# Chanuk-Yang/Deep_Continuous_Fusion_for_Multi-Sensor_3D_Object_Detection

Hardware: AMD Instinct MI355X
Metric: frames/sec (train step) 100k-pt LiDAR + 1242x375 RGB (higher is better)
Workload: dtype bf16; 1 GPU; cfg2: grid 32x704x800, 100000 pts/frame, 1242x375 RGB, ResNet-18 image stream, K=3 fusion x4 sites, eval-mode BN (reference F4), batch 2/GPU; global_batch=2, parallelism=dp1, loss_sampling=compat, conv_chain=False

## Files before the change

### deep_continuous_fusion_for_multi-sensor_3d_object_detection_amd/_hip.py

```python
import ctypes
import os
import subprocess

import numpy as np
import torch

_HERE = os.path.dirname(os.path.abspath(__file__))
LIB_PATH = os.environ.get("DCF_HIP_LIB") or os.path.join(_HERE, "libdcf_hip.so")
CSRC = os.path.join(_HERE, "csrc")

F32, BF16, F16 = 0, 1, 2
VOXEL_COMPAT, VOXEL_ACCUM, VOXEL_COMPAT_ROUNDS, VOXEL_OCCUPANCY = 0, 1, 2, 3
PROJ_COMPAT, PROJ_CORRECT = 0, 1

c_int, c_float, c_i64, c_size_t, c_void_p = ctypes.c_int, ctypes.c_float, ctypes.c_int64, ctypes.c_size_t, ctypes.c_void_p
P = c_void_p

SIGNATURES = {
    "dcf_last_error": (ctypes.c_char_p, []),
    "dcf_version": (c_int, []),
    "dcf_set_option": (c_int, [ctypes.c_char_p, ctypes.c_char_p]),
    "dcf_prof_enable": (c_int, [c_int]),
    "dcf_prof_reset": (c_int, []),
    "dcf_prof_calibrate": (c_int, [P, c_int]),
    "dcf_prof_read": (c_int, [P, P, P, P, c_int]),
    "dcf_prof_read2": (c_int, [P, P, P, P, P, c_int]),
    "dcf_compact_workspace_bytes": (c_size_t, [c_int]),
    "dcf_range_filter": (c_int, [P, c_int, P, P, P, P, P, P]),
    "dcf_voxelize_workspace_bytes": (c_size_t, [c_int, c_int, c_int]),
    "dcf_voxelize": (c_int, [P, c_int, P, P, c_int, c_int, c_int, c_int, P, P, P]),
    "dcf_voxelize_batch": (c_int, [P, P, c_int, P, P, c_int, c_int, c_int, P, P, P]),
    "dcf_voxelize_batch_nhwc": (c_int, [c_int, P, P, c_int, P, P, c_int, c_int, c_int, P, P, P]),
    "dcf_project_filter": (c_int, [P, c_int, P, P, c_float, c_float, c_int, P, P, P, P, P, P]),
    "dcf_project_filter_batch": (c_int, [P, P, c_int, P, P, c_float, c_float, c_int, P, P, c_int, P, P, P]),
    "dcf_knn_workspace_bytes": (c_size_t, [c_int, c_int, c_int]),
    "dcf_knn_bev": (c_int, [P, P, c_int, c_int, c_int, c_int, c_int, c_float, c_float, c_float, c_float, c_float, P, P, P]),
    "dcf_knn_bev_batch": (c_int, [P, P, c_int, c_int, c_int, c_int, c_int, c_int, c_float, c_float, c_float, c_float, c_float, P, P, c_size_t, P]),
    "dcf_knn_bev_sites": (c_int, [P, P, c_int, c_int, c_int, P, c_int, c_float, c_float, c_float, c_float, c_float, P]),
    "dcf_knn_bev_batch_shared": (c_int, [P, P, c_int, c_int, c_int, c_int, c_int, c_int, c_int, c_int, c_int, c_float, c_float, c_float, c_float, c_float, P, P, c_size_t, P, c_size_t, P]),
    "dcf_nchw_to_nhwc": (c_int, [c_int, P, P, c_int, c_int, c_int, c_int, P]),
    "dcf_nhwc_to_nchw": (c_int, [c_int, P, P, c_int, c_int, c_int, c_int, P]),
    "dcf_image_to_nhwc4": (c_int, [c_int, P, P, c_int, c_int, c_int, P]),
    "dcf_conv2d_fwd": (c_int, [c_int, P, P, P, P, P] + [c_int] * 12 + [P]),
    "dcf_conv2d_fwd_rowscale": (c_int, [c_int, P, P, P, P, P, P] + [c_int] * 12 + [P]),
    "dcf_conv2d_dgrad": (c_int, [c_int, P, P, P, P, P] + [c_int] * 11 + [P]),
    "dcf_conv2d_dgrad_halfres": (c_int, [c_int, P, P, P, P, P, P] + [c_int] * 11 + [P]),
    "dcf_conv3x3_chain_supported": (c_int, [c_int] * 6),
    "dcf_conv3x3_chain_workspace_bytes": (c_size_t, [c_int] * 6),
    "dcf_conv3x3_chain": (c_int, [c_int, P, c_int, c_int, c_int, c_int, c_int, c_int, P, P]),
    "dcf_fp8_act_scale": (c_int, [c_float, P]),
    "dcf_cast_fp8": (c_int, [c_int, P, P, P, P, c_i64, P]),
    "dcf_weight_prep_fp8": (c_int, [P, P, c_int, c_int, P, P, P, P, P, c_float, P]),
    "dcf_conv2d_fwd_fp8": (c_int, [c_int, P, P, P, P, P, P, P, P, P, P] + [c_int] * 12 + [P]),
    "dcf_conv2d_wgrad_splits": (c_int, [c_int] * 8),
    "dcf_conv2d_wgrad": (c_int, [c_int, P, P, P, P, c_int] + [c_int] * 11 + [P]),
    "dcf_conv2d_wgrad_groupable": (c_int, [c_int] * 10),
    "dcf_conv2d_wgrad_group": (c_int, [P, c_int, P]),
    "dcf_stem7x7_fwd": (c_int, [c_int, P, P, P, P] + [c_int] * 7 + [P]),
    "dcf_stem7x7_wgrad": (c_int, [c_int, P, P, P, P, c_int] + [c_int] * 6 + [P]),
    "dcf_weight_prep": (c_int, [c_int, P, c_int, P, P, P, P, c_float, P]),
    "dcf_wgrad_finalize": (c_int, [P, c_int, c_int, P, P, P, P, P, P, c_float, P]),
    "dcf_eval_score_filter": (c_int, [P, c_int, c_int, c_int, c_float, c_int, P, P, P]),
    "dcf_eval_nms_workspace_bytes": (c_size_t, [c_int]),
    "dcf_eval_nms": (c_int, [P, P, c_int, c_int, ctypes.c_double, P, P, P, P]),
    "dcf_eval_match": (c_int, [P, c_int, P, c_int, P, c_int, P, P]),
    "dcf_wgrad_finalize_rows": (c_int, [P, c_int, P, P, P, P, P, P, P, c_float, P]),
    "dcf_bn_workspace_bytes": (c_size_t, [c_int]),
    "dcf_bn_train_fwd": (c_int, [c_int, P, P, P, P, P, P, P, P, P, c_i64, c_int, c_float, c_float, c_int, P, P]),
    "dcf_bn_train_bwd": (c_int, [c_int, P, P, P, P, P, P, P, P, c_i64, c_int, P, P]),
    "dcf_relu_bwd_chansum": (c_int, [c_int, P, P, P, c_i64, c_int, c_int, P]),
    "dcf_resize_bilinear_fwd": (c_int, [c_int, P, P, P] + [c_int] * 7 + [P]),
    "dcf_resize_bilinear_bwd": (c_int, [c_int, P, P] + [c_int] * 7 + [P]),
    "dcf_maxpool3x3s2_fwd": (c_int, [c_int, P, P] + [c_int] * 6 + [P]),
    "dcf_maxpool3x3s2_bwd": (c_int, [c_int, P, P, P, P] + [c_int] * 6 + [P]),
    "dcf_maxpool3x3s2_fwd_idx": (c_int, [c_int, P, P, P] + [c_int] * 6 + [P]),
    "dcf_maxpool3x3s2_bwd_idx": (c_int, [c_int, P, P, P] + [c_int] * 6 + [P]),
    "dcf_head_fwd": (c_int, [c_int, P, c_int, P, P, c_int, c_int, c_int, P]),
    "dcf_head_bwd": (c_int, [c_int, P, c_int, P, P, P, P, c_int, c_int, c_int, P]),
    "dcf_point_sample_fwd": (c_int, [c_int, P, c_int, c_int, c_int, P, P, c_int, P, P]),
    "dcf_point_sample_bwd": (c_int, [c_int, P, c_int, c_int, c_int, P, P, c_int, P, P]),
    "dcf_point_sample_fwd_batch": (c_int, [c_int, P, c_int, c_int, c_int, P, c_i64, P, c_int, P, c_int, P]),
    "dcf_point_sample_bwd_batch": (c_int, [c_int, P, c_int, c_int, c_int, P, c_i64, P, c_int, P, c_int, P]),
    "dcf_fusion_gather_fwd_batch": (c_int, [c_int, P, c_i64, P, c_i64, P, c_int, c_int, c_int, c_int, c_float, c_float, c_float, c_float, P, P, c_int, P, P, c_int, P]),
    "dcf_fusion_gather_bwd_inv_batch": (c_int, [c_int, P, c_i64, P, c_i64, P, P, c_i64, P, P, c_int, c_int, c_int, c_int, c_float, c_float, c_float, c_float, P, P, c_int, P, P, P, P, P, c_int, P]),
    "dcf_fusion_gather_fwd": (c_int, [c_int, P, P, P, c_int, c_int, c_int, c_int, c_float, c_float, c_float, c_float, P, P, c_int, P, P, P]),
    "dcf_fusion_gather_bwd": (c_int, [c_int, P, P, P, c_int, c_int, c_int, c_int, c_float, c_float, c_float, c_float, P, P, c_int, P, P, P, P, P]),
    "dcf_fusion_invert_workspace_bytes": (c_size_t, [c_int, c_int]),
    "dcf_fusion_invert": (c_int, [P, c_int, c_int, c_int, P, P, P, P, P]),
    "dcf_fusion_gather_bwd_pts": (c_int, [c_int, P, P, P, c_int, P, P, c_int, c_int, c_int, c_int, c_float, c_float, c_float, c_float, P, P, c_int, P, P, P, P, P]),
    "dcf_fusion_gather_bwd_workspace_bytes": (c_size_t, [c_int]),
    "dcf_fusion_gather_bwd_direct_workspace_bytes": (c_size_t, [c_int, c_int, c_int]),
    "dcf_fusion_gather_bwd_direct_batch": (c_int, [c_int, P, c_i64, P, c_i64, P, P, c_i64, P, P, c_int, c_int, c_int, c_int, c_float, c_float, c_float, c_float, P, P, c_int, P, P, P, P, P, P, c_int, P]),
    "dcf_fusion_gather_bwd_inv": (c_int, [c_int, P, P, P, P, P, P, c_int, c_int, c_int, c_int, c_float, c_float, c_float, c_float, P, P, c_int, P, P, P, P, P, P]),
    "dcf_rowscale_bias_fwd": (c_int, [c_int, P, P, P, c_i64, c_int, P]),
    "dcf_rowscale_bias_bwd": (c_int, [c_int, P, P, P, c_i64, c_int, P]),
    "dcf_relu_mask_rowscale_bwd": (c_int, [c_int, P, P, P, P, P, c_i64, c_int, P]),
    "dcf_cast": (c_int, [c_int, P, c_int, P, c_i64, P]),
    "dcf_loss_fwd_bwd": (c_int, [P, c_i64, P, c_i64, P, P, P, c_int, c_int, c_float, c_int, P, P, c_i64, P, c_i64, P]),
    "dcf_loss_sample_rand": (ctypes.c_uint32, [ctypes.c_uint64, c_int, c_int, c_int, c_int]),
# ... 161 lines not shown
```

### deep_continuous_fusion_for_multi-sensor_3d_object_detection_amd/backend_hip.py

```python
import ctypes
import os

import numpy as np
import torch

from . import _hip as H
from . import ops

BN_EPS = 1e-5


class HipBackend(object):
    def __init__(self, plan, params, grads, buffers, dtype, fp8_min_cin=0, fp8_min_blocks=512):
        if not params.is_cuda:
            raise H.DcfError("the HIP hot path needs CUDA/HIP tensors (got %s); there is no CPU fallback" % params.device)
        H.lib()
        self.plan, self.params, self.grads, self.buffers = plan, params, grads, buffers
        self.dtype = H.dtype_code(dtype)
        self.tdtype = H.torch_dtype(self.dtype)
        self.es = 4 if self.dtype == H.F32 else 2
        self.dev = params.device
        self._fus_dws = {}
        self._wtab = {}
        self._chain_ok, self._chain_ws, self._chain_tab = {}, {}, {}
# ... 331 lines not shown
            import torch.distributed as dist
            if dist.is_available() and dist.is_initialized() and dist.get_world_size() > 1:
                return False
        key = tuple(shape)
        ok = self._chain_ok.get(key)
        if ok is None:
            B, Hh, W, C = key
            ok = self._chain_ok[key] = ops.conv3x3_chain_supported(self.dtype, B, Hh, W, C, 1)
        return ok

    def _chain(self, x, layers, flip):
        B, Hh, W, C = x.shape
        key = (B, Hh, W, C)
        ws = self._chain_ws.get(key)
        if ws is None:
            ws = self._chain_ws[key] = ops.conv3x3_chain_workspace(self.dtype, B, Hh, W, C, H.CHAIN_MAX_LAYERS, x.device)
        outs, cur, pos = [], x, 0
        while pos < len(layers):
            part = layers[pos:pos + H.CHAIN_MAX_LAYERS]
            fix = []
            for (w, sh, r, m, relu) in part:
                r = (outs[r] if r < pos else r - pos) if type(r) is int else r
                m = (outs[m] if m < pos else m - pos) if type(m) is int else m
                fix.append((w, sh, r, m, relu))
            tab = self._chain_tab.get(len(fix))
            if tab is None:
                tab = self._chain_tab[len(fix)] = (H.ChainLayer * len(fix))()
            got = ops.conv3x3_chain(self.dtype, cur, fix, flip, ws, tab)
            outs.extend(got)
            cur = got[-1]
            pos += len(part)
        return outs

    def chain_fwd(self, x, specs):
        outs = self._chain(x, [(self._wbase + L.wfwd_off, self._shift(L), r, None, relu) for (L, r, relu) in specs], 0)
        shp = (x.shape[0], x.shape[1], x.shape[2])
        for (L, _, _) in specs:
            L.out_shape = shp
        return outs

    def chain_dgrad(self, g, specs):
        for (L, _, _) in specs:
            if L.wdgrad_off < 0:
                raise H.DcfError("layer %s was planned without an input gradient" % L.name)
        return self._chain(g, [(self._wbase + L.wdgrad_off, None, r, m, False) for (L, r, m) in specs], 1)

    def shortcut_dgrad(self, Ld, dd, L1, g1, in_shape, mask=None):
        if L1.wdgrad_off < 0 or Ld.wdgrad_off < 0:
            raise H.DcfError("layer %s was planned without an input gradient" % L1.name)
        B, Hq, Wq, _ = dd.shape
        gq = ops.conv2d_dgrad(self.dtype, dd, self._w(Ld, True), None, (B, Hq, Wq, in_shape[3]), 1, 1, 1, 0)
        return ops.conv2d_dgrad_halfres(self.dtype, g1, self._w(L1, True), None, gq, in_shape, L1.kh, L1.kw, L1.stride, L1.pad, mask)

    def _gs(self, L):
        return self._gsbase + 4 * L.gsum_off if (L.bn is not None and not self.bn_train) else None

    def _flush_wgrads(self):
        q = self._wq
        if not q:
            return
        key = tuple([t[0].idx for t in q])
        ent = self._wtab.get(key)
        shapes = [t[1].shape for t in q]
        sig = (self.bn_train, self._slbase, self._gsbase, tuple([(t[0].nsplit, t[0].slab_off, t[0].gsum_off) for t in q]))
        if ent is None or ent[1] != shapes or ent[2] != sig:
            items = (H.WgradItem * len(q))()
            for i, (L, x, gy) in enumerate(q):
                B, Hh, W, Cin = x.shape
                items[i] = H.WgradItem(self.dtype, L.nsplit, 0, 0, self._slbase + 4 * L.slab_off, self._gs(L), B, Hh, W, Cin, L.cout_pad, L.kh, L.kw, L.stride, L.pad, 0)
            if len(self._wtab) > 16:
                self._wtab.clear()
            ent = self._wtab[key] = (items, shapes, sig)
        items = ent[0]
        for i, (L, x, gy) in enumerate(q):
            it = items[i]
            it.x = x.data_ptr()
            it.gy = gy.data_ptr()
        H.call("dcf_conv2d_wgrad_group", ctypes.addressof(items), len(q), H.stream_ptr())
        self._wq = []

    _wq = []
    _fus_ws = None
    _gp_pool = None
    _group = os.environ.get("DCF_WGRAD_GROUP", "1") != "0"
    _fusion_pts = os.environ.get("DCF_FUSION_PTS", "0") == "1"
    _fusion_direct = os.environ.get("DCF_FUSION_DIRECT", "1") != "0"

    def conv_wgrad(self, L, x, gy, defer=True):
        if self._group and defer and L.kind != "stem":
            q = self.__dict__.get("_wq")
            if q is None:
                q = self._wq = []
            q.append((L, x, gy))
            return
        ops.conv2d_wgrad(self.dtype, x, gy, self._slbase + 4 * L.slab_off, L.nsplit, L.kh, L.kw, L.stride, L.pad, self._gs(L))

    def stem_fwd(self, L, img4, Hh, W):
        if self.bn_train:
            raw = ops.stem7x7_fwd(self.dtype, img4, self._w(L), None, False, L.cout_pad, Hh, W)
            L.out_shape = (raw.shape[0], raw.shape[1], raw.shape[2])
            return self._bn_fwd(L, raw, None, True)
        y = ops.stem7x7_fwd(self.dtype, img4, self._w(L), self._shift(L), True, L.cout_pad, Hh, W)
        L.out_shape = (y.shape[0], y.shape[1], y.shape[2])
        return y

    def stem_wgrad(self, L, img4, gy, Hh, W):
# ... 145 lines not shown
```

### deep_continuous_fusion_for_multi-sensor_3d_object_detection_amd/engine.py

```python
import os

import numpy as np
import torch

FUSION_INV = os.environ.get("DCF_FUSION_INV", "1")
FUSED_SITE_MASK = os.environ.get("DCF_FUSED_SITE_MASK", "1") != "0"
HALFRES_SHORTCUT = os.environ.get("DCF_HALFRES_SHORTCUT", "1") != "0"


class ConvLayer(object):

    def __init__(self, idx, name, cin, cout, kh, kw, stride, pad, bn=None, kind="conv", need_dgrad=True, names=None):
        self.idx, self.name, self.bn, self.kind = idx, name, bn, kind
        self.cin, self.cout, self.kh, self.kw, self.stride, self.pad = cin, cout, kh, kw, stride, pad
        self.cout_pad = (cout + 31) // 32 * 32
        self.need_dgrad = need_dgrad
        self.names = names or [name]
        self.w_off = self.gamma_off = self.beta_off = self.mean_off = self.var_off = -1
        self.out_shape = None

    @property
    def taps(self):
        return self.kh * self.kw


class ParamTable(object):

    def __init__(self):
        self.entries = []
        self.buffers = []
        self.n_params = 0
        self.n_buffers = 0

    def add_param(self, key, shape, layout="plain"):
        n = int(np.prod(ParamTable.physical_shape(shape, layout)))
        off = self.n_params
        self.entries.append((key, tuple(shape), off, n, layout))
        self.n_params += (n + 3) // 4 * 4
        return off

    def add_buffer(self, key, shape):
        n = int(np.prod(shape)) if len(shape) else 1
        off = self.n_buffers
        self.buffers.append((key, tuple(shape), off, n))
        self.n_buffers += (n + 3) // 4 * 4
        return off

    @staticmethod
    def physical_shape(shape, layout):
        if layout == "ohwi":
            O, I, kh, kw = shape
            return (O, kh, kw, I)
        if layout == "stem":
            return (shape[0], 7, 8, 4)
        return tuple(shape)

    @staticmethod
    def view(flat, shape, off, n, layout):
        seg = flat[off:off + n]
        if layout == "ohwi":
            O, I, kh, kw = shape
            return seg.view(O, kh, kw, I).permute(0, 3, 1, 2)
        if layout == "stem":
            return seg.view(shape[0], 7, 8, 4)[:, :, :7, :3].permute(0, 3, 1, 2)
        return seg.view(shape)


class Block(object):

    def __init__(self, conv1, conv2, down=None):
        self.conv1, self.conv2, self.down = conv1, conv2, down
        self.saved = None
        self.next_conv = None

    def forward(self, K, x, save=True):
        r = K.conv_fwd(self.down, x, None, False) if self.down is not None else x
        y1 = K.conv_fwd(self.conv1, x, None, True, self.conv2)
        y = K.conv_fwd(self.conv2, y1, r, True, self.next_conv)
        x._f8 = y1._f8 = None
        self.saved = (x, y1, y) if save else None
        return y

    def backward(self, K, g, extra=None, need_gx=True, g_masked=False, prev=None):
        x, y1, y = self.saved
        self.saved = None
        g2 = g if g_masked else K.relu_mask(g, y)
        d2 = K.bn_bwd(self.conv2, g2)
        K.conv_wgrad(self.conv2, y1, d2)
        g1 = K.bn_bwd(self.conv1, K.conv_dgrad(self.conv2, d2, tuple(y1.shape), None, y1))
        return self.backward_tail(K, x, g2, g1, extra, need_gx, prev)

    def backward_tail(self, K, x, g2, g1, extra, need_gx, prev):
        K.conv_wgrad(self.conv1, x, g1)
        pm = x if prev is not None else None
        if self.down is not None:
            dd = K.bn_bwd(self.down, g2)
            K.conv_wgrad(self.down, x, dd)
            if not need_gx:
                return None
            d, c = self.down, self.conv1
            if (extra is None and HALFRES_SHORTCUT and d.kh == 1 and d.kw == 1 and d.stride == 2 and d.pad == 0
                    and c.kh == 3 and c.stride == 2 and c.pad == 1):
                return K.shortcut_dgrad(d, dd, c, g1, tuple(x.shape), pm)
            gx = K.conv_dgrad(self.down, dd, tuple(x.shape), extra)
            return K.conv_dgrad(self.conv1, g1, tuple(x.shape), gx, pm)
        if not need_gx:
            return None
        assert extra is None, "an identity-shortcut block cannot take an extra gradient"
        return K.conv_dgrad(self.conv1, g1, tuple(x.shape), g2, pm)


def blocks_forward(K, blocks, x, save=True):
    n = len(blocks)
    ok = (n >= 1 and getattr(K, "can_chain", None) is not None and all(type(b) is Block for b in blocks)
          and all(b.down is None and b.conv1.stride == 1 for b in blocks[1:]))
    if ok:
        b0 = blocks[0]
        strided = b0.down is not None or b0.conv1.stride != 1 or b0.conv1.cin != b0.conv1.cout
        nchain = 2 * n - 1 if strided else 2 * n
        B, Hh, W, _ = x.shape
        s0 = b0.conv1.stride
        shape = (B, (Hh + 2 - 3) // s0 + 1, (W + 2 - 3) // s0 + 1, b0.conv1.cout) if strided else tuple(x.shape)
        ok = nchain >= 2 and all(L.kh == 3 and L.kw == 3 and L.pad == 1 and L.cout == L.cout_pad == shape[3]
                                 for b in blocks for L in (b.conv1, b.conv2)) and K.can_chain(shape, nchain)
    if not ok:
        for b in blocks:
            x = b.forward(K, x, save)
        return x
    specs, ins = [], []
    if strided:
        r = K.conv_fwd(b0.down, x, None, False) if b0.down is not None else x
        y1 = K.conv_fwd(b0.conv1, x, None, True)
        x0 = y1
        specs.append((b0.conv2, r, True))
        first = 1
    else:
        x0 = x
        first = 0
    xin = len(specs) - 1
    for b in blocks[first:]:
        specs.append((b.conv1, None, True))
        specs.append((b.conv2, xin if xin >= 0 else x, True))
        xin = len(specs) - 1
    outs = K.chain_fwd(x0, specs)
    if save:
        k = 0
        if strided:
            b0.saved = (x, y1, outs[0])
            k = 1
        prev = outs[0] if strided else x
        for b in blocks[first:]:
            b.saved = (prev, outs[k], outs[k + 1])
            prev = outs[k + 1]
# ... 489 lines not shown
```

### deep_continuous_fusion_for_multi-sensor_3d_object_detection_amd/ops.py

```python
import ctypes

import numpy as np
import torch

from . import _hip as H


def _chk(t, name):
    if not (isinstance(t, torch.Tensor) and t.is_cuda and t.is_contiguous()):
        raise H.DcfError("%s must be a contiguous CUDA tensor" % name)
    return t


def conv_out_size(n, k, s, p):
    return (n + 2 * p - k) // s + 1


def nchw_to_nhwc(x, dtype):
    B, C, Hh, W = x.shape
    _chk(x, "x")
    y = torch.empty((B, Hh, W, C), dtype=H.torch_dtype(dtype), device=x.device)
    H.call("dcf_nchw_to_nhwc", dtype, x, y, B, C, Hh, W, H.stream_ptr())
    return y

# ... 22 lines not shown
    H.call("dcf_conv2d_fwd", dtype, x, w, shift, res, y, B, Hh, W, Cin, Ho, Wo, cout, kh, kw, stride, pad, int(relu),
           H.stream_ptr())
    return y


def conv2d_fwd_rowscale(dtype, x, w, shift, rowscale, res, relu, cout):
    B, Hh, W, Cin = x.shape
    if rowscale.numel() != B * Hh * W or rowscale.dtype != torch.float32:
        raise H.DcfError("conv2d_fwd_rowscale: rowscale must be fp32 with one entry per output pixel")
    y = torch.empty((B, Hh, W, cout), dtype=x.dtype, device=x.device)
    H.call("dcf_conv2d_fwd_rowscale", dtype, x, w, shift, _chk(rowscale, "rowscale"), res, y, B, Hh, W, Cin, Hh, W, cout, 1, 1, 1, 0, int(relu),
           H.stream_ptr())
    return y


def fp8_act_scale(amax):
    import ctypes
    out = ctypes.c_float(0.0)
    H.call("dcf_fp8_act_scale", float(amax), ctypes.addressof(out))
    return float(out.value)


def cast_fp8(dtype, x, amax_prev=None, amax_cur=None):
    x8 = torch.empty(x.shape, dtype=torch.uint8, device=x.device)
    H.call("dcf_cast_fp8", dtype, x, x8, amax_prev, amax_cur, x.numel(), H.stream_ptr())
    return x8


def conv2d_fwd_fp8(out_dtype, x8, w8, wscale, xamax, shift, res, kh, kw, stride, pad, relu, cout, want_y8=False, y8amax=None, y8cur=None):
    B, Hh, W, Cin = x8.shape
    Ho, Wo = conv_out_size(Hh, kh, stride, pad), conv_out_size(W, kw, stride, pad)
    y = torch.empty((B, Ho, Wo, cout), dtype=H.torch_dtype(out_dtype), device=x8.device)
    y8 = torch.empty((B, Ho, Wo, cout), dtype=torch.uint8, device=x8.device) if want_y8 else None
    H.call("dcf_conv2d_fwd_fp8", out_dtype, x8, w8, wscale, xamax, shift, res, y, y8, y8amax, y8cur, B, Hh, W, Cin, Ho, Wo, cout, kh, kw,
           stride, pad, int(relu), H.stream_ptr())
    return (y, y8) if want_y8 else y


def conv2d_dgrad(dtype, gy, wt, res, in_shape, kh, kw, stride, pad, mask=None):
    B, Hh, W, Cin = in_shape
    _, Ho, Wo, Cout = gy.shape
    gx = torch.empty((B, Hh, W, Cin), dtype=gy.dtype, device=gy.device)
    H.call("dcf_conv2d_dgrad", dtype, gy, wt, res, mask, gx, B, Hh, W, Cin, Ho, Wo, Cout, kh, kw, stride, pad, H.stream_ptr())
    return gx


def conv2d_dgrad_halfres(dtype, gy, wt, res, resq, in_shape, kh, kw, stride, pad, mask=None):
    B, Hh, W, Cin = in_shape
    _, Ho, Wo, Cout = gy.shape
    if tuple(resq.shape) != (B, (Hh + 1) // 2, (W + 1) // 2, Cin):
        raise H.DcfError("conv2d_dgrad_halfres: resq %s does not sit on the even sub-grid of %s" % (tuple(resq.shape), tuple(in_shape)))
    gx = torch.empty((B, Hh, W, Cin), dtype=gy.dtype, device=gy.device)
    H.call("dcf_conv2d_dgrad_halfres", dtype, gy, wt, res, resq, mask, gx, B, Hh, W, Cin, Ho, Wo, Cout, kh, kw, stride, pad, H.stream_ptr())
    return gx


def conv3x3_chain_supported(dtype, B, Hh, W, C, nlayers):
    return bool(H.lib().dcf_conv3x3_chain_supported(dtype, B, Hh, W, C, nlayers))


def conv3x3_chain_workspace(dtype, B, Hh, W, C, nlayers, device):
    n = H.lib().dcf_conv3x3_chain_workspace_bytes(dtype, B, Hh, W, C, nlayers)
    if n == 0:
        raise H.DcfError("conv3x3_chain: unsupported shape %s x %d layers" % ((B, Hh, W, C), nlayers))
    return torch.zeros((n // 4,), dtype=torch.int32, device=device)


def conv3x3_chain(dtype, x, layers, flip, ws, table=None):
    B, Hh, W, C = x.shape
    n = len(layers)
    outs = [torch.empty((B, Hh, W, C), dtype=x.dtype, device=x.device) for _ in range(n)]
    tab = table if table is not None else (H.ChainLayer * n)()
    cur = x.data_ptr()
    for l, (w, shift, res, mask, relu) in enumerate(layers):
        it = tab[l]
        it.x = cur
        it.w = H._ptr(w)
        it.shift = H._ptr(shift)
        it.res = outs[res].data_ptr() if type(res) is int else H._ptr(res)
        it.mask = outs[mask].data_ptr() if type(mask) is int else H._ptr(mask)
        cur = it.y = outs[l].data_ptr()
        it.relu = 1 if relu else 0
    import ctypes
    H.call("dcf_conv3x3_chain", dtype, ctypes.addressof(tab), n, B, Hh, W, C, int(flip), ws, H.stream_ptr())
    return outs


def conv3x3_chain_status(ws):
    return int(ws[1].item())


def conv2d_wgrad_splits(B, Ho, Wo, Cin, Cout, kh, kw, stride=1):
    return H.lib().dcf_conv2d_wgrad_splits(B, Ho, Wo, Cin, Cout, kh, kw, stride)


def conv2d_wgrad(dtype, x, gy, slabs, nsplit, kh, kw, stride, pad, gsum=None):
    B, Hh, W, Cin = x.shape
    _, Ho, Wo, Cout = gy.shape
    H.call("dcf_conv2d_wgrad", dtype, x, gy, slabs, gsum, nsplit, B, Hh, W, Cin, Ho, Wo, Cout, kh, kw, stride, pad, H.stream_ptr())
    return slabs


def stem7x7_fwd(dtype, img4, w, shift, relu, cout, Hh, W):
    B = img4.shape[0]
    Ho, Wo = conv_out_size(Hh, 7, 2, 3), conv_out_size(W, 7, 2, 3)
    y = torch.empty((B, Ho, Wo, cout), dtype=img4.dtype, device=img4.device)
# ... 460 lines not shown
```

### include/dcf_hip.h

```cpp
#ifndef DCF_HIP_H
#define DCF_HIP_H

#include <stddef.h>
#include <stdint.h>

#ifdef __cplusplus
extern "C" {
#endif

typedef void *dcf_stream_t;

enum { DCF_OK = 0, DCF_EINVAL = -1, DCF_ELAUNCH = -2, DCF_EUNSUPPORTED = -3 };
enum { DCF_F32 = 0, DCF_BF16 = 1, DCF_F16 = 2 };
enum { DCF_VOXEL_COMPAT = 0, DCF_VOXEL_ACCUM = 1, DCF_VOXEL_COMPAT_ROUNDS = 2,
       DCF_VOXEL_OCCUPANCY = 3  };
enum { DCF_PROJ_COMPAT = 0, DCF_PROJ_CORRECT = 1 };

const char *dcf_last_error(void);
int dcf_version(void);
int dcf_set_option(const char *name, const char *value);
int dcf_prof_enable(int on);
int dcf_prof_reset(void);
int dcf_prof_calibrate(dcf_stream_t stream, int n);
int dcf_prof_read(char *names , double *total_ms, int64_t *calls, double *work, int cap);
// ... 8 lines not shown
int dcf_voxelize(const float *pts, int n, const float *lim, const float *aff, int Cz, int L, int W,
                 int mode, float *grid, void *owner_ws, dcf_stream_t stream);
#define DCF_MAX_VOXEL_BATCH 8
int dcf_voxelize_batch(const float *const *pts, const int *n, int B, const float *lim, const float *aff, int Cz, int L, int W,
                       float *grids, void *owner_ws, dcf_stream_t stream);
int dcf_voxelize_batch_nhwc(int dtype, const float *const *pts, const int *n, int B, const float *lim, const float *aff, int Cz, int L,
                            int W, void *x_nhwc, void *owner_ws, dcf_stream_t stream);

int dcf_project_filter(const float *pts, int n, const float *lim, const float *crt, float ulim, float vlim,
                       int mode, float *uv_out, float *xyz_out, int32_t *src_out, int32_t *count_dev,
                       void *ws, dcf_stream_t stream);
int dcf_project_filter_batch(const float *const *pts, const int *n, int B, const float *lim, const float *crt, float ulim, float vlim,
                             int mode, float *uv_out, float *xyz_out, int rows, int32_t *count_dev, void *ws, dcf_stream_t stream);

size_t dcf_knn_workspace_bytes(int n_max, int h, int w);
int dcf_knn_bev(const float *xyz, const int32_t *count_dev, int n_max, int K, int h, int w, int stride,
                float xs, float xo, float ys, float yo, float rmax2, int32_t *idx_out, void *ws,
                dcf_stream_t stream);
int dcf_knn_bev_batch(const float *xyz, const int32_t *count_dev, int B, int n_max, int K, int h, int w, int stride,
                      float xs, float xo, float ys, float yo, float rmax2, int32_t *idx_out, void *ws, size_t ws_stride_bytes,
                      dcf_stream_t stream);

int dcf_knn_bev_batch_shared(const float *xyz, const int32_t *count_dev, int B, int n_max, int K, int h, int w, int stride,
                             int fine_h, int fine_w, int fine_stride, float xs, float xo, float ys, float yo, float rmax2,
                             int32_t *idx_out, void *ws, size_t ws_stride_bytes, const void *ws_fine, size_t ws_fine_stride_bytes,
                             dcf_stream_t stream);

typedef struct { int32_t h, w, stride, fine; int32_t *idx_out; void *ws; size_t ws_stride_bytes; } dcf_knn_site;
int dcf_knn_bev_sites(const float *xyz, const int32_t *count_dev, int B, int n_max, int K, const dcf_knn_site *sites, int nsites,
                      float xs, float xo, float ys, float yo, float rmax2, dcf_stream_t stream);

#define DCF_MAX_KNN_MAPS 32
typedef struct { const int32_t *idx; int32_t h, w; } dcf_knn_map;
size_t dcf_fusion_invert_workspace_bytes(int n_max, int nmaps);
int dcf_fusion_invert(const dcf_knn_map *maps, int nmaps, int K, int n_max, int32_t *start, int32_t *ent_pix, int32_t *ent_pt,
                      void *ws, dcf_stream_t stream);

int dcf_nchw_to_nhwc(int dtype, const float *x, void *y, int B, int C, int H, int W, dcf_stream_t stream);
int dcf_nhwc_to_nchw(int dtype, const void *x, float *y, int B, int C, int H, int W, dcf_stream_t stream);
int dcf_image_to_nhwc4(int dtype, const uint8_t *img, void *y, int B, int H, int W, dcf_stream_t stream);

int dcf_conv2d_fwd(int dtype, const void *x, const void *w, const float *shift, const void *res, void *y,
                   int B, int H, int W, int Cin, int Ho, int Wo, int Cout, int kh, int kw, int stride, int pad,
                   int relu, dcf_stream_t stream);
int dcf_conv2d_fwd_rowscale(int dtype, const void *x, const void *w, const float *shift, const float *rowscale, const void *res,
                            void *y, int B, int H, int W, int Cin, int Ho, int Wo, int Cout, int kh, int kw, int stride, int pad,
                            int relu, dcf_stream_t stream);
int dcf_conv2d_dgrad(int dtype, const void *gy, const void *wt, const void *res, const void *mask, void *gx,
                     int B, int H, int W, int Cin, int Ho, int Wo, int Cout, int kh, int kw, int stride, int pad,
                     dcf_stream_t stream);
int dcf_conv2d_dgrad_halfres(int dtype, const void *gy, const void *wt, const void *res, const void *resq,
                             const void *mask, void *gx, int B, int H, int W, int Cin, int Ho, int Wo, int Cout,
                             int kh, int kw, int stride, int pad, dcf_stream_t stream);
#define DCF_CHAIN_MAX_LAYERS 24
typedef struct {
    const void *x, *w;
    const float *shift;
    const void *res, *mask;
    void *y;
    int32_t relu, pad_;
} dcf_chain_layer;
int dcf_conv3x3_chain_supported(int dtype, int B, int H, int W, int C, int nlayers);
size_t dcf_conv3x3_chain_workspace_bytes(int dtype, int B, int H, int W, int C, int nlayers);
int dcf_conv3x3_chain(int dtype, const dcf_chain_layer *layers, int nlayers, int B, int H, int W, int C, int flip,
                      void *ws, dcf_stream_t stream);
int dcf_conv2d_wgrad_splits(int B, int Ho, int Wo, int Cin, int Cout, int kh, int kw, int stride);
int dcf_conv2d_wgrad(int dtype, const void *x, const void *gy, float *slabs, float *gsum, int nsplit,
                     int B, int H, int W, int Cin, int Ho, int Wo, int Cout, int kh, int kw, int stride, int pad,
                     dcf_stream_t stream);
typedef struct {
    int32_t dtype, nsplit;
    const void *x, *gy;
    float *slabs, *gsum;
    int32_t B, H, W, Cin, Cout, kh, kw, stride, pad, pad_;
} dcf_wgrad_item;
int dcf_conv2d_wgrad_groupable(int dtype, int B, int H, int W, int Cin, int Cout, int kh, int kw, int stride, int pad);
int dcf_conv2d_wgrad_group(const dcf_wgrad_item *items, int n, dcf_stream_t stream);
int dcf_stem7x7_fwd(int dtype, const void *img4, const void *w, const float *shift, void *y,
                    int B, int H, int W, int Ho, int Wo, int Cout, int relu, dcf_stream_t stream);
int dcf_stem7x7_wgrad(int dtype, const void *img4, const void *gy, float *slabs, float *gsum, int nsplit,
                      int B, int H, int W, int Ho, int Wo, int Cout, dcf_stream_t stream);

typedef struct dcf_conv_param {
    int64_t w_off;
    int64_t gamma_off;
    int64_t beta_off;
    int64_t mean_off;
    int64_t var_off;
    int64_t wfwd_off;
    int64_t wdgrad_off;
    int64_t shift_off;
    int64_t slab_off;
    int64_t gsum_off;
    int32_t cout, cin, taps, cout_pad;
    int32_t nsplit, flags, pad0, pad1;
} dcf_conv_param;
int dcf_weight_prep(int dtype, const dcf_conv_param *table, int nconv, const float *params, const float *buffers,
                    void *warena, float *ssarena, float eps, dcf_stream_t stream);
int dcf_wgrad_finalize(const dcf_conv_param *table, int nconv, int max_cout, const float *params, const float *buffers,
                       const float *ssarena, const float *slabs, const float *gsum, float *grads, float eps,
                       dcf_stream_t stream);
int dcf_wgrad_finalize_rows(const dcf_conv_param *table, int nconv, const int32_t *cout_host, const float *params, const float *buffers,
                            const float *ssarena, const float *slabs, const float *gsum, float *grads, float eps,
                            dcf_stream_t stream);

int dcf_fp8_act_scale(float amax, float *scale);
// ... 111 lines not shown
```

Measured before the change: 384.7 frames/s.

## Fuse stride-2 block head dgrad with 1x1 shortcut dgrad in one kernel

Adds a dedicated HIP kernel that computes the input gradient of a stride-2 residual block head in a single pass. It combines the 3x3 stride-2 conv dgrad, the 1x1 stride-2 downsample dgrad, the optional extra residual add and the ReLU mask. Work is split by output parity class across waves, with weights held in registers and tiles double- or triple-buffered through LDS with async loads. The aim is to remove the separate quarter-res dgrad kernel, its intermediate tensor and the extra launch. In exchange it adds a complex specialised kernel limited to 32->64 and 64->128 channels in 16-bit types.

```diff
diff --git a/deep_continuous_fusion_for_multi-sensor_3d_object_detection_amd/_hip.py b/deep_continuous_fusion_for_multi-sensor_3d_object_detection_amd/_hip.py
--- a/deep_continuous_fusion_for_multi-sensor_3d_object_detection_amd/_hip.py
+++ b/deep_continuous_fusion_for_multi-sensor_3d_object_detection_amd/_hip.py
@@ -45,6 +45,7 @@
     "dcf_conv2d_fwd_rowscale": (c_int, [c_int, P, P, P, P, P, P] + [c_int] * 12 + [P]),
     "dcf_conv2d_dgrad": (c_int, [c_int, P, P, P, P, P] + [c_int] * 11 + [P]),
     "dcf_conv2d_dgrad_halfres": (c_int, [c_int, P, P, P, P, P, P] + [c_int] * 11 + [P]),
+    "dcf_conv2d_s2head_dgrad": (c_int, [c_int, P, P, P, P, P, P, P] + [c_int] * 7 + [P]),
     "dcf_conv3x3_chain_supported": (c_int, [c_int] * 6),
     "dcf_conv3x3_chain_workspace_bytes": (c_size_t, [c_int] * 6),
     "dcf_conv3x3_chain": (c_int, [c_int, P, c_int, c_int, c_int, c_int, c_int, c_int, P, P]),
diff --git a/deep_continuous_fusion_for_multi-sensor_3d_object_detection_amd/backend_hip.py b/deep_continuous_fusion_for_multi-sensor_3d_object_detection_amd/backend_hip.py
--- a/deep_continuous_fusion_for_multi-sensor_3d_object_detection_amd/backend_hip.py
+++ b/deep_continuous_fusion_for_multi-sensor_3d_object_detection_amd/backend_hip.py
@@ -407,6 +407,17 @@
         gq = ops.conv2d_dgrad(self.dtype, dd, self._w(Ld, True), None, (B, Hq, Wq, in_shape[3]), 1, 1, 1, 0)
         return ops.conv2d_dgrad_halfres(self.dtype, g1, self._w(L1, True), None, gq, in_shape, L1.kh, L1.kw, L1.stride, L1.pad, mask)
 
+    def s2head_ok(self, L1, Ld, in_shape):
+        return (self.dtype != H.F32 and L1.kh == 3 and L1.kw == 3 and L1.stride == 2 and L1.pad == 1
+                and Ld.kh == 1 and Ld.kw == 1 and Ld.stride == 2 and Ld.pad == 0
+                and (L1.cin, L1.cout) in ((32, 64), (64, 128)) and L1.cout == L1.cout_pad
+                and Ld.cin == L1.cin and Ld.cout == L1.cout and in_shape[3] == L1.cin)
+
+    def s2head_dgrad(self, L1, Ld, g1, dd, in_shape, extra=None, mask=None):
+        if L1.wdgrad_off < 0 or Ld.wdgrad_off < 0:
+            raise H.DcfError("layer %s was planned without an input gradient" % L1.name)
+        return ops.conv2d_s2head_dgrad(self.dtype, g1, self._w(L1, True), dd, self._w(Ld, True), extra, in_shape, mask)
+
     def _gs(self, L):
         return self._gsbase + 4 * L.gsum_off if (L.bn is not None and not self.bn_train) else None
 
diff --git a/deep_continuous_fusion_for_multi-sensor_3d_object_detection_amd/csrc/conv_s2.hip b/deep_continuous_fusion_for_multi-sensor_3d_object_detection_amd/csrc/conv_s2.hip
--- /dev/null
+++ b/deep_continuous_fusion_for_multi-sensor_3d_object_detection_amd/csrc/conv_s2.hip
@@ -0,0 +1,336 @@
+#include <stdlib.h>
+
+#include <algorithm>
+#include <type_traits>
+
+#include "dcf_common.h"
+#include "conv_common.h"
+
+namespace {
+
+struct S2Args {
+    const char *g;
+    const char *w;
+    const char *dd;
+    const char *wd;
+    const char *extra;
+    const char *mask;
+    char *gx;
+    int B, H, W, Ho, Wo;
+    int txn, tyn, ntiles;
+    unsigned gbytes, xbytes;
+};
+
+typedef unsigned s2_u32x4 __attribute__((ext_vector_type(4)));
+
+template <int CI, int CO, int TH, int NBUF>
+struct S2Cfg {
+    static constexpr int NW = CI / 32 * 4;
+    static constexpr int RB = CO * 2;
+    static constexpr int CPP = RB / 16;
+    static constexpr int PPP = 1024 / RB;
+    static constexpr int GR = TH / 2 + 1;
+    static constexpr int PW = CO == 64 ? 18 : 17;
+    static constexpr int NPG = (GR * PW + PPP - 1) / PPP;
+    static constexpr int DR = TH / 2;
+    static constexpr int NPD = DR * 16 / PPP;
+    static constexpr int NPIECE = NPG + NPD;
+    static constexpr int PXW = (NPIECE + NW - 1) / NW;
+    static constexpr int TMT = TH / 4;
+    static constexpr int KS = CO / 16;
+    static constexpr int NST = TMT * 2;
+    static constexpr int DUMP = NBUF * NPIECE;
+    static constexpr int AHEAD = (NBUF - 2) * (PXW + NST) + NST;
+    static constexpr int LDS = (NBUF * NPIECE + 1) * 1024;
+    static_assert(CO == 64 || CO == 128, "64 or 128 gradient channels");
+    static_assert(TH % 4 == 0 && (PW * RB) % 256 == 0 && (16 * RB) % 256 == 0 && (DR * 16) % PPP == 0, "tile shape");
+    static_assert(NBUF >= 2 && AHEAD < 64, "vmcnt range");
+    static_assert(LDS * (CI == 32 ? 2 : 1) <= 160 * 1024, "LDS: two workgroups per CU (one with eight waves)");
+};
+
+template <int CO> __device__ __forceinline__ int s2_key(int cc) { return CO == 64 ? (cc >> 1) & 7 : cc & 15; }
+
+template <typename T> __device__ __forceinline__ float s2_round(float v);
+template <> __device__ __forceinline__ float s2_round<bf16_t>(float v) { return bf2f(f2bf(v)); }
+template <> __device__ __forceinline__ float s2_round<f16_t>(float v) { return h2f(f2h(v)); }
+
+template <typename T, int CI, int CO, int TH, int NBUF, int CLS>
+__device__ __forceinline__ void s2_dgrad_wave(const S2Args &a, char *lds, const int wid, int t, const int chunk_hi, const int wpx)
+{
+    using C = S2Cfg<CI, CO, TH, NBUF>;
+    constexpr int RB = C::RB, CPP = C::CPP, PPP = C::PPP, PW = C::PW, KS = C::KS, TMT = C::TMT, NPG = C::NPG, NPIECE = C::NPIECE;
+    constexpr int PH = CLS >> 1, PC = CLS & 1;
+    constexpr int NR = PH ? 2 : 1, NC = PC ? 2 : 1, NT = NR * NC;
+    const int lane = threadIdx.x & 63, r = lane & 31, h = lane >> 5;
+    const int n0 = (wid >> 2) * 32;
+    const __amdgpu_buffer_rsrc_t srcG = __builtin_amdgcn_make_buffer_rsrc((void *)a.g, 0, a.gbytes, 0x00020000);
+    const __amdgpu_buffer_rsrc_t srcD = __builtin_amdgcn_make_buffer_rsrc((void *)a.dd, 0, a.gbytes, 0x00020000);
+    const __amdgpu_buffer_rsrc_t dstX = __builtin_amdgcn_make_buffer_rsrc((void *)a.gx, 0, a.xbytes, 0x00020000);
+    constexpr unsigned OOB = 0xFFFFFF00u;
+    const unsigned lds0 = lds_addr(lds);
+
+    uint4 wreg[NT * KS];
+    uint4 wdr[CLS == 0 ? KS : 1];
+    {
+        const char *wp = a.w + (size_t)(n0 + r) * (9 * RB) + h * 16;
+#pragma unroll
+        for (int u = 0; u < NR; ++u)
+#pragma unroll
+            for (int v = 0; v < NC; ++v) {
+                const int ki = PH ? (u ? 2 : 0) : 1, kj = PC ? (v ? 2 : 0) : 1;
+#pragma unroll
+                for (int ks = 0; ks < KS; ++ks) wreg[(u * NC + v) * KS + ks] = *reinterpret_cast<const uint4 *>(wp + (ki * 3 + kj) * RB + ks * 32);
+            }
+        if constexpr (CLS == 0) {
+#pragma unroll
+            for (int ks = 0; ks < KS; ++ks) wdr[ks] = *reinterpret_cast<const uint4 *>(a.wd + (size_t)(n0 + r) * RB + h * 16 + ks * 32);
+        }
+    }
+
+    auto piece_px = [&](int p, int ln, int &rr_, int &cc_) __attribute__((always_inline)) {
+        if (p < NPG) { const int i = p * PPP + ln / CPP; rr_ = i / PW; cc_ = i - rr_ * PW; return i < C::GR * PW && cc_ < 17; }
+        const int i = (p - NPG) * PPP + ln / CPP; rr_ = i >> 4; cc_ = i & 15; return p < NPIECE;
+    };
+    int relo[C::PXW];
+#pragma unroll
+    for (int j = 0; j < C::PXW; ++j) {
+        int rr_, cc_;
+        const bool ok = piece_px(wid + C::NW * j, lane, rr_, cc_);
+        relo[j] = ok ? (rr_ * a.Wo + cc_) * RB + (((lane % CPP) ^ s2_key<CO>(cc_)) << 4) : -1;
+    }
+    auto issue_tile = [&](int tile, int buf) __attribute__((always_inline)) {
+        const int tx = tile % a.txn, tq = tile / a.txn;
+        const int ty = tq % a.tyn, b = tq / a.tyn;
+        const int a0 = ty * (TH / 2), b0 = tx * 16;
+        const bool inner = tile < chunk_hi && a0 + C::GR <= a.Ho && b0 + 17 <= a.Wo;
+        const int org = ((b * a.Ho + a0) * a.Wo + b0) * RB;
+#pragma unroll
+        for (int j = 0; j < C::PXW; ++j) {
+            const int p = wid + C::NW * j;
+            bool live = relo[j] >= 0;
+            if (!inner) {
+                int rr_, cc_;
+                piece_px(p, opaque(lane), rr_, cc_);
+                live = live && tile < chunk_hi && a0 + rr_ < a.Ho && b0 + cc_ < a.Wo;
+            }
+            glds16(p < NPG ? srcG : srcD, live ? (unsigned)(org + relo[j]) : OOB,
+                   __builtin_amdgcn_readfirstlane(lds0 + (p < NPIECE ? buf * NPIECE + p : C::DUMP) * 1024));
+        }
+    };
+
+    const int ri = r >> 4, cj = r & 15;
+    int goff[NC][KS];
+#pragma unroll
+    for (int v = 0; v < NC; ++v) {
+        const int dj = PC ? (v ? 0 : 1) : 0;
+#pragma unroll
+        for (int ks = 0; ks < KS; ++ks) goff[v][ks] = ri * PW * RB + (cj + dj) * RB + (((2 * ks + h) ^ s2_key<CO>(cj + dj)) << 4);
+    }
+    int doff[CLS == 0 ? KS : 1];
+    if constexpr (CLS == 0) {
+#pragma unroll
+        for (int ks = 0; ks < KS; ++ks) doff[ks] = NPG * 1024 + (ri * 16 + cj) * RB + (((2 * ks + h) ^ s2_key<CO>(cj)) << 4);
+    }
+
+    const T *extra = reinterpret_cast<const T *>(a.extra);
+    const T *mask = reinterpret_cast<const T *>(a.mask);
+    const int c0 = n0 + 8 * h;
+
+#pragma unroll
+    for (int d = 0; d < NBUF - 1; ++d) {
+        issue_tile(t + d * wpx, d);
+#pragma unroll
+        for (int k = 0; k < C::NST; ++k) {
+            const s2_u32x4 z = {0u, 0u, 0u, 0u};
+            asm volatile("buffer_store_dwordx4 %0, %1, %2, 0 offen\n\ts_nop 1" ::"v"(z), "v"(OOB), "s"(dstX) : "memory");
+        }
+    }
+    int buf = 0;
+    for (;;) {
+        const int tx = t % a.txn, tq = t / a.txn;
+        const int ty = tq % a.tyn, b = tq / a.tyn;
+        const int tn = t + wpx;
+        wait_vmcnt<C::AHEAD>();
+        asm volatile("s_waitcnt lgkmcnt(0)" ::: "memory");
+        __builtin_amdgcn_s_barrier();
+        issue_tile(t + (NBUF - 1) * wpx, buf == 0 ? NBUF - 1 : buf - 1);
+        const char *slot = lds + buf * (NPIECE * 1024);
+        f32x16 acc[TMT], accd[CLS == 0 ? TMT : 1];
+#pragma unroll
+        for (int j = 0; j < TMT; ++j)
+#pragma unroll
+            for (int q = 0; q < 16; ++q) acc[j][q] = 0.f;
+#pragma unroll
+        for (int u = 0; u < NR; ++u)
+#pragma unroll
+            for (int v = 0; v < NC; ++v) {
+                const int di = PH ? (u ? 0 : 1) : 0;
+                asm volatile("" ::: "memory");
+#pragma unroll
+                for (int ks = 0; ks < KS; ++ks) {
+                    uint4 fb[TMT];
+#pragma unroll
+                    for (int j = 0; j < TMT; ++j) fb[j] = *reinterpret_cast<const uint4 *>(slot + goff[v][ks] + (2 * j + di) * PW * RB);
+#pragma unroll
+                    for (int j = 0; j < TMT; ++j) Mma<T>::run(wreg[(u * NC + v) * KS + ks], fb[j], acc[j]);
+                }
+            }
+        if constexpr (CLS == 0) {
+#pragma unroll
+            for (int j = 0; j < TMT; ++j)
+#pragma unroll
+                for (int q = 0; q < 16; ++q) accd[j][q] = 0.f;
+            asm volatile("" ::: "memory");
+#pragma unroll
+            for (int ks = 0; ks < KS; ++ks) {
+                uint4 fb[TMT];
+#pragma unroll
+                for (int j = 0; j < TMT; ++j) fb[j] = *reinterpret_cast<const uint4 *>(slot + doff[ks] + 2 * j * 16 * RB);
+#pragma unroll
+                for (int j = 0; j < TMT; ++j) Mma<T>::run(wdr[ks], fb[j], accd[j]);
+            }
+        }
+        int m[TMT];
+#pragma unroll
+        for (int j = 0; j < TMT; ++j) {
+            const int yy = ty * TH + 2 * (2 * j + ri) + PH, xx = tx * 32 + 2 * cj + PC;
+            m[j] = (yy < a.H && xx < a.W) ? (b * a.H + yy) * a.W + xx : -1;
+            acc_rows8(acc[j]);
+            if constexpr (CLS == 0) acc_rows8(accd[j]);
+        }
+        if (extra) {
+            uint4 ee[TMT][2];
+#pragma unroll
+            for (int j = 0; j < TMT; ++j)
+#pragma unroll
+                for (int p = 0; p < 2; ++p)
+                    ee[j][p] = m[j] >= 0 ? *reinterpret_cast<const uint4 *>(extra + (size_t)m[j] * CI + c0 + 16 * p) : make_uint4(0, 0, 0, 0);
+#pragma unroll
+            for (int j = 0; j < TMT; ++j)
+#pragma unroll
+                for (int p = 0; p < 2; ++p) {
+                    const unsigned ew[4] = {ee[j][p].x, ee[j][p].y, ee[j][p].z, ee[j][p].w};
+#pragma unroll
+                    for (int e = 0; e < 4; ++e) {
+                        float lo, hi;
+                        unpack2<T>(ew[e], lo, hi);
+                        if constexpr (CLS == 0) {
+                            accd[j][8 * p + 2 * e] += lo; accd[j][8 * p + 2 * e + 1] += hi;
+                        } else {
+                            acc[j][8 * p + 2 * e] += lo; acc[j][8 * p + 2 * e + 1] += hi;
+                        }
+                    }
+                }
+        }
+        if constexpr (CLS == 0) {
+#pragma unroll
+            for (int j = 0; j < TMT; ++j)
+#pragma unroll
+                for (int k = 0; k < 16; ++k) acc[j][k] += s2_round<T>(accd[j][k]);
+        }
+        if (mask) {
+            uint4 mm[TMT][2];
+#pragma unroll
+            for (int j = 0; j < TMT; ++j)
+#pragma unroll
+                for (int p = 0; p < 2; ++p)
+                    mm[j][p] = m[j] >= 0 ? *reinterpret_cast<const uint4 *>(mask + (size_t)m[j] * CI + c0 + 16 * p) : make_uint4(0, 0, 0, 0);
+#pragma unroll
+            for (int j = 0; j < TMT; ++j)
+#pragma unroll
+                for (int p = 0; p < 2; ++p) {
+                    const unsigned mw[4] = {mm[j][p].x, mm[j][p].y, mm[j][p].z, mm[j][p].w};
+#pragma unroll
+                    for (int e = 0; e < 4; ++e) {
+                        float lo, hi;
+                        unpack2<T>(mw[e], lo, hi);
+                        if (!(lo > 0.f)) acc[j][8 * p + 2 * e] = 0.f;
+                        if (!(hi > 0.f)) acc[j][8 * p + 2 * e + 1] = 0.f;
+                    }
+                }
+        }
+#pragma unroll
+        for (int j = 0; j < TMT; ++j)
+#pragma unroll
+            for (int p = 0; p < 2; ++p) {
+                float v[8];
+#pragma unroll
+                for (int k = 0; k < 8; ++k) v[k] = acc[j][8 * p + k];
+                uint4 pk;
+                if constexpr (std::is_same<T, bf16_t>::value) {
+                    pk = make_uint4(pack2bf(v[0], v[1]), pack2bf(v[2], v[3]), pack2bf(v[4], v[5]), pack2bf(v[6], v[7]));
+                } else {
+                    typedef _Float16 h16x8 __attribute__((ext_vector_type(8)));
+                    h16x8 hv;
+#pragma unroll
+                    for (int k = 0; k < 8; ++k) hv[k] = (_Float16)v[k];
+                    pk = __builtin_bit_cast(uint4, hv);
+                }
+                const s2_u32x4 d = {pk.x, pk.y, pk.z, pk.w};
+                __builtin_amdgcn_raw_buffer_store_b128(d, dstX, m[j] >= 0 ? (int)((unsigned)(m[j] * CI + c0 + 16 * p) * 2u) : (int)OOB, 0, 0);
+            }
+        if (tn >= chunk_hi) break;
+        t = tn;
+        buf = buf + 1 == NBUF ? 0 : buf + 1;
+    }
+}
+
+template <typename T, int CI, int CO, int TH, int NBUF>
+__global__ void __launch_bounds__(CI / 32 * 256) __attribute__((amdgpu_waves_per_eu(2, 2))) k_conv_s2h_dgrad(S2Args a)
+{
+    static_assert(DT<T>::size == 2, "16-bit element types only");
+    __shared__ __attribute__((aligned(1024))) char lds[S2Cfg<CI, CO, TH, NBUF>::LDS];
+    const int wid = __builtin_amdgcn_readfirstlane(threadIdx.x >> 6);
+    const int chunk = (a.ntiles + 7) >> 3;
+    const int wpx = gridDim.x >> 3;
+    const int chunk_lo = (blockIdx.x & 7) * chunk, chunk_hi = min(chunk_lo + chunk, a.ntiles);
+    const int t = chunk_lo + (blockIdx.x >> 3);
+    if (t >= chunk_hi) return;
+    switch (wid & 3) {
+    case 0: s2_dgrad_wave<T, CI, CO, TH, NBUF, 0>(a, lds, wid, t, chunk_hi, wpx); break;
+    case 1: s2_dgrad_wave<T, CI, CO, TH, NBUF, 1>(a, lds, wid, t, chunk_hi, wpx); break;
+    case 2: s2_dgrad_wave<T, CI, CO, TH, NBUF, 2>(a, lds, wid, t, chunk_hi, wpx); break;
+    default: s2_dgrad_wave<T, CI, CO, TH, NBUF, 3>(a, lds, wid, t, chunk_hi, wpx); break;
+    }
+}
+
+}
+
+extern "C" int dcf_conv2d_s2head_dgrad(int dtype, const void *g1, const void *wt, const void *dd, const void *wdt, const void *extra,
+                                       const void *mask, void *gx, int B, int H, int W, int Cin, int Ho, int Wo, int Cout,
+                                       dcf_stream_t stream)
+{
+    if (!(dtype == DCF_BF16 || dtype == DCF_F16) || !((Cin == 32 && Cout == 64) || (Cin == 64 && Cout == 128))) {
+        dcf_set_error("dcf_conv2d_s2head_dgrad: 16-bit types with 32 -> 64 or 64 -> 128 channels only (dtype %d, %d -> %d)", dtype, Cin, Cout);
+        return DCF_EUNSUPPORTED;
+    }
+    DCF_REQUIRE(g1 && wt && dd && wdt && gx, "dcf_conv2d_s2head_dgrad: null pointer");
+    DCF_REQUIRE(B >= 1 && H >= 1 && W >= 1 && Ho == (H - 1) / 2 + 1 && Wo == (W - 1) / 2 + 1, "dcf_conv2d_s2head_dgrad: output size mismatch");
+    DCF_REQUIRE((int64_t)B * H * W * Cin * 2 < 0x7FFFFF00ll, "dcf_conv2d_s2head_dgrad: tensor too large for 32-bit offsets");
+    S2Args a;
+    a.g = (const char *)g1; a.w = (const char *)wt; a.dd = (const char *)dd; a.wd = (const char *)wdt;
+    a.extra = (const char *)extra; a.mask = (const char *)mask; a.gx = (char *)gx;
+    a.B = B; a.H = H; a.W = W; a.Ho = Ho; a.Wo = Wo;
+    const int TH = Cin == 32 ? 16 : 8;
+    a.txn = (W + 31) / 32; a.tyn = (H + TH - 1) / TH;
+    a.ntiles = B * a.txn * a.tyn;
+    a.gbytes = (unsigned)((int64_t)B * Ho * Wo * Cout * 2);
+    a.xbytes = (unsigned)((int64_t)B * H * W * Cin * 2);
+    const int wgpc = Cin == 32 ? 2 : 1;
+    const int64_t nwg = std::min<int64_t>(((int64_t)a.ntiles + 7) / 8 * 8, 256 * wgpc);
+    const dim3 grid((unsigned)nwg), block(Cin / 32 * 256);
+    const double hw = (double)B * Ho * Wo;
+    const double flops = 2.0 * hw * Cout * Cin * 10.0;
+    const double bytes = 2.0 * hw * Cout * 2.0 + (double)B * H * W * Cin * 2.0 * (1 + (extra ? 1 : 0) + (mask ? 1 : 0)) + 10.0 * Cin * Cout * 2.0;
+    const char *name = dtype == DCF_F16 ? (Cin == 32 ? "conv_dgrad_f16<s2h32>" : "conv_dgrad_f16<s2h64>")
+                                        : (Cin == 32 ? "conv_dgrad_bf16<s2h32>" : "conv_dgrad_bf16<s2h64>");
+    hipStream_t s = S(stream);
+#define DCF_S2(T_)                                                                                                                 \
+    do {                                                                                                                           \
+        if (Cin == 32) DCF_LAUNCH_WB(name, flops, bytes, s, hipLaunchKernelGGL((k_conv_s2h_dgrad<T_, 32, 64, 16, 2>), grid, block, 0, s, a)); \
+        else DCF_LAUNCH_WB(name, flops, bytes, s, hipLaunchKernelGGL((k_conv_s2h_dgrad<T_, 64, 128, 8, 3>), grid, block, 0, s, a));          \
+    } while (0)
+    if (dtype == DCF_F16) DCF_S2(f16_t); else DCF_S2(bf16_t);
+#undef DCF_S2
+    return DCF_OK;
+}
diff --git a/deep_continuous_fusion_for_multi-sensor_3d_object_detection_amd/engine.py b/deep_continuous_fusion_for_multi-sensor_3d_object_detection_amd/engine.py
--- a/deep_continuous_fusion_for_multi-sensor_3d_object_detection_amd/engine.py
+++ b/deep_continuous_fusion_for_multi-sensor_3d_object_detection_amd/engine.py
@@ -6,6 +6,7 @@
 FUSION_INV = os.environ.get("DCF_FUSION_INV", "1")
 FUSED_SITE_MASK = os.environ.get("DCF_FUSED_SITE_MASK", "1") != "0"
 HALFRES_SHORTCUT = os.environ.get("DCF_HALFRES_SHORTCUT", "1") != "0"
+S2HEAD = os.environ.get("DCF_S2HEAD", "1") != "0"
 
 
 class ConvLayer(object):
@@ -99,6 +100,8 @@
             if not need_gx:
                 return None
             d, c = self.down, self.conv1
+            if S2HEAD and getattr(K, "s2head_ok", None) is not None and K.s2head_ok(c, d, tuple(x.shape)):
+                return K.s2head_dgrad(c, d, g1, dd, tuple(x.shape), extra, pm)
             if (extra is None and HALFRES_SHORTCUT and d.kh == 1 and d.kw == 1 and d.stride == 2 and d.pad == 0
                     and c.kh == 3 and c.stride == 2 and c.pad == 1):
                 return K.shortcut_dgrad(d, dd, c, g1, tuple(x.shape), pm)
diff --git a/deep_continuous_fusion_for_multi-sensor_3d_object_detection_amd/ops.py b/deep_continuous_fusion_for_multi-sensor_3d_object_detection_amd/ops.py
--- a/deep_continuous_fusion_for_multi-sensor_3d_object_detection_amd/ops.py
+++ b/deep_continuous_fusion_for_multi-sensor_3d_object_detection_amd/ops.py
@@ -98,6 +98,16 @@
         raise H.DcfError("conv2d_dgrad_halfres: resq %s does not sit on the even sub-grid of %s" % (tuple(resq.shape), tuple(in_shape)))
     gx = torch.empty((B, Hh, W, Cin), dtype=gy.dtype, device=gy.device)
     H.call("dcf_conv2d_dgrad_halfres", dtype, gy, wt, res, resq, mask, gx, B, Hh, W, Cin, Ho, Wo, Cout, kh, kw, stride, pad, H.stream_ptr())
+    return gx
+
+
+def conv2d_s2head_dgrad(dtype, g1, wt, dd, wdt, extra, in_shape, mask=None):
+    B, Hh, W, Cin = in_shape
+    _, Ho, Wo, Cout = g1.shape
+    if tuple(dd.shape) != tuple(g1.shape):
+        raise H.DcfError("conv2d_s2head_dgrad: dd %s and g1 %s differ" % (tuple(dd.shape), tuple(g1.shape)))
+    gx = torch.empty((B, Hh, W, Cin), dtype=g1.dtype, device=g1.device)
+    H.call("dcf_conv2d_s2head_dgrad", dtype, g1, wt, dd, wdt, extra, mask, gx, B, Hh, W, Cin, Ho, Wo, Cout, H.stream_ptr())
     return gx
 
 
diff --git a/include/dcf_hip.h b/include/dcf_hip.h
--- a/include/dcf_hip.h
+++ b/include/dcf_hip.h
@@ -84,6 +84,9 @@
 int dcf_conv2d_dgrad_halfres(int dtype, const void *gy, const void *wt, const void *res, const void *resq,
                              const void *mask, void *gx, int B, int H, int W, int Cin, int Ho, int Wo, int Cout,
                              int kh, int kw, int stride, int pad, dcf_stream_t stream);
+int dcf_conv2d_s2head_dgrad(int dtype, const void *g1, const void *wt, const void *dd, const void *wdt, const void *extra,
+                            const void *mask, void *gx, int B, int H, int W, int Cin, int Ho, int Wo, int Cout,
+                            dcf_stream_t stream);
 #define DCF_CHAIN_MAX_LAYERS 24
 typedef struct {
     const void *x, *w;
```

Measured after the change: 389.2 frames/s (median of 6 runs). 1.01x the previous value.
